# TFMV/hnsw

Hardware: AMD Instinct MI355X
Metric: queries/sec @ recall@10, 1M×768-d cosine; 1/2/4/8-GPU scaling (higher is better)
Workload: dtype fp32

## Files before the change

hnsw_amd/csrc/api.cpp:

```cpp
#include "index.hpp"

#include <functional>
#include <unordered_set>

using namespace mhh;

namespace mhh {

thread_local std::string g_create_err;

int fail(mhnsw_index* h, int code, const char* fmt, ...) {
    char buf[512];
    va_list ap;
    va_start(ap, fmt);
    vsnprintf(buf, sizeof(buf), fmt, ap);
    va_end(ap);
    if (h)
        h->err = buf;
    else
        g_create_err = buf;
    return code;
}

int validate(mhnsw_index* h) {
// ... 317 lines not shown
            h->ord_pin = nullptr;
            h->ord_cap = 0;
            if (hipHostMalloc((void**)&h->ord_pin, (size_t)nb * 4, hipHostMallocDefault) != hipSuccess)
                return fail(h, MHNSW_ENOMEM, "pinned allocation failed");
            h->ord_cap = nb;
        }
        if ((r = ensure_buf(h, h->border, (size_t)nb))) return r;
        if (h->ord_pending) HIPCHK(h, hipEventSynchronize(h->ord_ev));
        std::vector<int64_t> pos(MH_MAXL + 1, 0);
        for (int l = 0; l <= MH_MAXL; ++l) pos[l] = l < MH_MAXL ? count[l + 1] : 0;
        for (int64_t i = a0; i < a1; ++i)
            h->ord_pin[pos[std::min(h->hlevels[row_of(i)], MH_MAXL)]++] = (uint32_t)row_of(i);
        HIPCHK(h, hipMemcpyAsync(h->border.p, h->ord_pin, (size_t)nb * 4, hipMemcpyHostToDevice, h->stream));
        HIPCHK(h, hipEventRecord(h->ord_ev, h->stream));
        h->ord_pending = true;
    }
    auto vis16_for = [&](int ef) -> int {
        return h->vis_compact && ef > 128 && h->capn <= (int64_t(1) << 24) && h->vis_log2 == 12;
    };
    auto args = [&](int l) {
        const int mcap = l == 0 ? m0_of(h) : h->M;
        BatchBuildArgs a;
        a.order = nullptr;
        a.count = 0;
        a.g = graph_view(h);
        a.layer = l;
        a.n0 = rows ? 0 : a0;
        a.n1 = rows ? nb : a1;
        a.rows = rows ? h->border.p : nullptr;
        a.levels = h->levels;
// ... 30 lines not shown
        if (!h->time_build) return 0;
        if (h->ltev_used == h->ltev.size()) {
            hipEvent_t e;
            HIPCHK(h, hipEventCreate(&e));
            h->ltev.push_back(e);
        }
        HIPCHK(h, hipEventRecord(h->ltev[h->ltev_used++], h->stream));
        return 0;
    };
    for (int l = top; l >= 0; --l) {
        BatchBuildArgs a = args(l);
        const int mcap = a.mcap;
        if (fuse) {
            if (l == top) {
                if ((r = tmark())) return r;
                LCHK(h, launch_build_batch_descend(a, h->lpr, h->vpl, h->stream));
                if ((r = tmark())) return r;
            }
            if (l > maxlvl) continue;
            a.order = h->border.p;
            a.count = count[std::min(l, MH_MAXL)];
        }
        HIPCHK(h, hipMemsetAsync(h->touched_cnt, 0, 4, h->stream));
        if ((r = tmark())) return r;
        LCHK(h, launch_build_batch_search(a, h->lpr, h->vpl, h->stream));
        if (maxlvl >= l) LCHK(h, launch_build_batch_commit(a, h->lpr, h->vpl, (a1 - a0) * mcap, h->stream));
        if ((r = tmark())) return r;
        if (link && count[std::min(l, MH_MAXL)] >= 2) {
            if ((size_t)nb > h->link_cap || h->link_stride < h->layers[l].cap)
                return fail(h, MHNSW_EINTERNAL, "link staging too small");
            BatchBuildArgs la = a;
            la.ef = h->batch_link_ef > 0 ? std::min(std::max(h->batch_link_ef, mcap), 512) : a.ef;
            la.vis16 = vis16_for(la.ef);
            LinkArgs k;
            k.adj = h->link_adj;
            k.adjd = h->link_adjd;
// ... 564 lines not shown
        r = run_build_batch(h, n0, n1, top_live, entry_live, publish_keys);
        publish_keys();
    }
    HIPCHK(h, hipStreamSynchronize(h->stream));
    if (int rt = collect_build_times(h)) return rt;
    if (r == 0) *reached = nproc;
    *cont_out = cont;
    return r;
}

int add_impl(mhnsw_index* h, const int64_t* keys, const float* vecs, bool vecs_on_device, int64_t n, int dim,
             const int32_t* levels) {
    h->add_reached = 0;
    h->link_rows = h->link_edges = 0;
    h->link_us = 0;
    for (;;) {
        int64_t reached = 0, cont = -1;
        const int r = add_step(h, keys, vecs, vecs_on_device, n, dim, levels, &reached, &cont);
        h->add_reached += reached;
        if (r || cont <= 0 || cont >= n) return r;
        keys += cont;
        vecs += (size_t)cont * dim;
        n -= cont;
        if (levels) levels += cont;
    }
}

}

extern "C" {
// ... 76 lines not shown
        F(L.adj);
        F(L.adjd);
    }
    F(h->qpad.p);
    F(h->qnorm.p);
    F(h->scores.p);
    F(h->tmp.p);
    F(h->cand.p);
    F(h->border.p);
    F(h->okeys.p);
    F(h->odist.p);
    F(h->on.p);
    F(h->ordkey.p);
    F(h->ordval.p);
    F(h->ordtmp.p);
    F(h->nq.p);
    F(h->nneg.p);
    F(h->ncd.p);
    F(h->nck.p);
    F(h->nok.p);
    F(h->ncn.p);
    F(h->nci.p);
    F(h->noff.p);
    F(h->non.p);
    F(h->nos.p);
    F(h->xsplit.p);
    F(h->xinv.p);
    F(h->qinv.p);
    F(h->xerr.p);
    F(h->h1thr.p);
// ... 196 lines not shown
    } else if (n == "build_mw_max") {
        if (v < 0) return fail(h, MHNSW_EINVAL, "build_mw_max must be >= 0");
        h->build_mw_max = v;
    } else if (n == "beam_mw_max_b") {
        if (v < 0) return fail(h, MHNSW_EINVAL, "beam_mw_max_b must be >= 0");
        h->beam_mw_max_b = v;
    } else if (n == "beam_lds_min_ef") {
        if (v < 65 || v > 513) return fail(h, MHNSW_EINVAL, "beam_lds_min_ef must be in [65, 513]");
        h->beam_lds_min_ef = (int)v;
    } else if (n == "upper_ef") {
        if (v < 1 || v > 64) return fail(h, MHNSW_EINVAL, "upper_ef must be in [1, 64]");
        h->upper_ef = (int)v;
    } else if (n == "fuse_descent") {
        if (v != 0 && v != 1) return fail(h, MHNSW_EINVAL, "fuse_descent must be 0 or 1");
        h->fuse_descent = (int)v;
    } else if (n == "vis_compact") {
        if (v != 0 && v != 1) return fail(h, MHNSW_EINVAL, "vis_compact must be 0 or 1");
        h->vis_compact = (int)v;
    } else if (n == "filter_route") {
        if (v < 1 || v > 2048) return fail(h, MHNSW_EINVAL, "filter_route must be in [1, 2048]");
        h->filter_route = (int)v;
    } else if (n == "compact_stage_rows") {
        if (v < 1) return fail(h, MHNSW_EINVAL, "compact_stage_rows must be >= 1");
        h->compact_stage_rows = v;
    } else if (n == "time_build") {
        h->time_build = (int)(v != 0);
    } else if (n == "max_rows") {
        if (v < 0) return fail(h, MHNSW_EINVAL, "max_rows must be >= 0");
        h->max_rows = v;
    } else if (n == "screen") {
// ... 57 lines not shown
    else if (n == "batch_ratio_pct") *v = h->batch_ratio_pct;
    else if (n == "vis_log2") *v = h->vis_log2;
    else if (n == "vis_entries") *v = beam_vis_entries(h);
    else if (n == "exact_kk") *v = h->exact_kk;
    else if (n == "exact_sample") *v = h->exact_sample;
    else if (n == "exact_thr_rank") *v = h->exact_thr_rank;
    else if (n == "exact_precision") *v = h->exact_precision;
    else if (n == "exact_tile") *v = h->exact_tile;
    else if (n == "compat_waves") *v = h->compat_waves;
    else if (n == "upper_ef") *v = h->upper_ef;
    else if (n == "beam_mw_max_b") *v = h->beam_mw_max_b;
    else if (n == "beam_lds_min_ef") *v = h->beam_lds_min_ef;
    else if (n == "build_mw_max") *v = h->build_mw_max;
    else if (n == "screen") *v = h->screen;
    else if (n == "fuse_descent") *v = h->fuse_descent;
    else if (n == "vis_compact") *v = h->vis_compact;
    else if (n == "filter_route") *v = h->filter_route;
    else if (n == "time_build") *v = h->time_build;
    else if (n == "max_rows") *v = h->max_rows;
    else if (n == "strkey_relabels") *v = h->relabels;
    else if (n == "strkeys") *v = (int64_t)h->s2l.size();
    else if (n == "pitch") *v = h->pitch;
    else if (n == "capacity") *v = h->capn;
    else if (n == "last_gemm_ns") {
        float ms = 0.f;
        if (!h->have_gemm_timing || hipEventSynchronize(h->gev1) != hipSuccess ||
            hipEventElapsedTime(&ms, h->gev0, h->gev1) != hipSuccess)
            return MHNSW_EINVAL;
        *v = (int64_t)std::llround((double)ms * 1e6);
    }
// ... 485 lines not shown
    if (!relink && n > 0 && (!keys || !vecs || !out_found))
        return fail(h, MHNSW_EINVAL, "keys, vecs and out_found must be non-NULL");
    if (h->build_mode == MHNSW_BUILD_COMPAT || h->aliased || h->partial_rows > 0)
        return fail(h, MHNSW_EUNSUPPORTED, "update needs a batch or flat (build_mode 1 or 2) handle");
    if (n <= 0) return MHNSW_OK;
    if (!relink && h->layers_exist && dim != h->dim)
        return fail(h, MHNSW_EDIM, "embedding dimension mismatch: %d != %d", h->dim, dim);
    {
        std::unordered_set<int64_t> seen;
        seen.reserve((size_t)n);
        for (int64_t i = 0; i < n; ++i)
            if (!seen.insert(keys[i]).second)
                return fail(h, MHNSW_EINVAL, "duplicate key %lld in update", (long long)keys[i]);
    }
    h->update_rows = h->update_chunks = h->update_repaired = 0;
    h->update_us[0] = h->update_us[1] = h->update_us[2] = 0;
    std::vector<uint32_t> ids, from;
    for (int64_t i = 0; i < n; ++i) {
        out_found[i] = 0;
        auto it = h->key2id.find(keys[i]);
        if (it == h->key2id.end() || h->hdead[it->second] || !in_layer(h, it->second, 0)) continue;
        out_found[i] = 1;
        ids.push_back((uint32_t)it->second);
        from.push_back((uint32_t)i);
    }
    const int64_t m = (int64_t)ids.size();
    if (m == 0) return MHNSW_OK;
    ++h->mut_epoch;
    const bool flat = h->build_mode == MHNSW_BUILD_FLAT;
    hipStream_t s = h->stream;
// ... 437 lines not shown
```

hnsw_amd/csrc/beam.hpp:

```cpp
#pragma once
#include <type_traits>

#include "device_search.hpp"
#include "engine.hpp"

namespace mh {

template <int L, int V, int XW>
int launch_beam_cfg(const SearchArgs& a, hipStream_t s);
template <int L, int V, int XW>
int launch_beam_lds_cfg(const SearchArgs& a, hipStream_t s);
template <int L, int V>
int launch_beam_filt_cfg(const SearchArgs& a, const FilterArgs& f, hipStream_t s);

__host__ __device__ inline int beam_efl(const SearchArgs& a) { return a.ef > a.k ? a.ef : a.k; }
inline bool beam_in_lds(const SearchArgs& a) { return beam_efl(a) >= a.lds_min_ef; }

__host__ __device__ inline int beam_vis_words(const SearchArgs& a) { return a.vis16 ? VIS16_WORDS : a.vis_n; }

struct BeamLds {
    int list, words;
};
template <class LT>
__host__ __device__ inline BeamLds beam_lds(const SearchArgs& a) {
// ... 28 lines not shown
                const int32_t e = a.layer_entry[l];
                if (e < 0)
                    skip = true;
                else
                    ep = (uint32_t)e;
            }
            if (!skip) {
                beam_layer<C, 1, G, false, SCREEN, 1>(a.g, l, ep, a.upper_ef, q, qn, L1, smem, vsz, st, bev);
                float d;
                uint32_t id;
                bl_at(L1, 0, d, id);
                if (id != EMPTY_ID) ep = id & ID_MASK;
            }
            if constexpr (KEY) {
                if (l <= a.key_top && l > a.key_top - a.key_n) {
                    const uint32_t f = a.key_hash ? (ep * 2654435761u) >> (32 - a.key_id_bits)
                                                  : ep & ((1u << a.key_id_bits) - 1u);
                    *key = (*key << a.key_id_bits) | (unsigned long long)f;
                }
            }
        }
    }
    if (to0 && a.g.layers[0].deg[ep] == -2) ep = (uint32_t)a.layer_entry[0];
    return ep;
}

__device__ __forceinline__ uint32_t beam_entry_of(const SearchArgs& a, int64_t b) {
    return a.order ? uni(a.ep0[b]) : a.entry;
}
__device__ __forceinline__ int beam_entry_layer(const SearchArgs& a) { return a.order ? beam_order_lo(a) - 1 : a.top; }

__device__ __forceinline__ void beam_pad_out(const SearchArgs& a, int64_t b, int nvalid) {
    const int lane = lane_id();
// ... 58 lines not shown
        const bool ok = w != EMPTY_ID && !is_dead(a.g, id);
        const unsigned long long m = __ballot(ok);
        const int pos = nvalid + __popcll(m & below);
        if (ok && pos < a.k) {
            a.out_keys[b * a.k + pos] = a.g.keys[id];
            a.out_dist[b * a.k + pos] = bl_chunk_dist(L, c);
            if (a.out_ids) a.out_ids[b * a.k + pos] = (int32_t)id;
        }
        nvalid += __popcll(m);
    }
    beam_pad_out(a, b, min(nvalid, a.k));
}

__device__ __forceinline__ int64_t beam_query_of(const SearchArgs& a, int64_t i) {
    if (!a.order) return i < a.B ? i : -1;
    const int64_t pos = a.order_chunk > 0 ? (i & 7) * a.order_chunk + (i >> 3) : i;
    if (pos >= a.B || (a.order_chunk > 0 && (i >> 3) >= a.order_chunk)) return -1;
    const uint32_t b = uni(a.order[pos]);
    return b < (uint64_t)a.B ? (int64_t)b : -1;
}

__device__ __forceinline__ void beam_stats(const SearchArgs& a, const WaveStats& st) {
    if (lane_id() == 0) {
        atomicAdd(&a.stats[0], st.E);
        atomicAdd(&a.stats[1], st.X);
        if (st.resets) atomicAdd(&a.stats[2], st.resets);
        atomicAdd(&a.stats[8], st.S);
        atomicAdd(&a.stats[9], st.F);
#ifdef MH_PROF_BEAM
        atomicAdd(&a.stats[10], st.c_ins);
        atomicAdd(&a.stats[11], st.c_score);
// ... 212 lines not shown
```

hnsw_amd/csrc/build.hip:

```cpp
#include "build_batch.hpp"
#include "build_link.hpp"
#include "build_compat.hpp"

namespace mh {
#define X_(L, V, G)                                                                           \
    extern template int launch_build_compat_cfg<L, V>(const CompatBuildArgs&, int, hipStream_t); \
    extern template int launch_delete_compat_cfg<L, V>(const DeleteArgs&, hipStream_t);       \
    extern template int launch_batch_descend_cfg<L, V>(const BatchBuildArgs&, hipStream_t);   \
    extern template int launch_batch_search_cfg<L, V, 1>(const BatchBuildArgs&, hipStream_t); \
    extern template int launch_batch_search_cfg<L, V, 2>(const BatchBuildArgs&, hipStream_t); \
    extern template int launch_batch_search_cfg<L, V, 3>(const BatchBuildArgs&, hipStream_t); \
    extern template int launch_batch_search_cfg<L, V, 4>(const BatchBuildArgs&, hipStream_t); \
    extern template int launch_batch_commit_cfg<L, V>(const BatchBuildArgs&, int64_t, hipStream_t); \
    extern template int launch_batch_link_cfg<L, V, 1>(const BatchBuildArgs&, const LinkArgs&, hipStream_t); \
    extern template int launch_batch_link_cfg<L, V, 2>(const BatchBuildArgs&, const LinkArgs&, hipStream_t); \
    extern template int launch_batch_link_cfg<L, V, 3>(const BatchBuildArgs&, const LinkArgs&, hipStream_t); \
    extern template int launch_batch_link_cfg<L, V, 4>(const BatchBuildArgs&, const LinkArgs&, hipStream_t); \
    extern template int launch_delete_repair_cfg<L, V>(const DeleteArgs&, hipStream_t);
MH_FOR_EACH_CFG(X_)
#undef X_

int launch_build_compat(const CompatBuildArgs& a, int lpr, int vpl, int waves, hipStream_t s) {
    return with_cfg(lpr, vpl, [&](auto c) { return launch_build_compat_cfg<c.L, c.V>(a, waves, s); });
}
// ... 46 lines not shown
    if (keep) {
        c = k.adj[(size_t)slot * k.stride + lane];
        d = k.adjd[(size_t)slot * k.stride + lane];
        for (int j = 0; j < nin; ++j) keep = keep && a.inc_src[(size_t)u * a.inc_cap + j] != (uint32_t)c;
    }
    const unsigned long long m = __ballot(keep);
    if (keep) {
        const int e = __builtin_amdgcn_mbcnt_hi((uint32_t)(m >> 32), __builtin_amdgcn_mbcnt_lo((uint32_t)m, 0));
        a.g.layers[l].adj[(size_t)u * capl + e] = c;
        a.g.layers[l].adjd[(size_t)u * capl + e] = d;
    }
    if (lane == 0) a.g.layers[l].deg[u] = __popcll(m);
}

int launch_build_batch_link_apply(const BatchBuildArgs& a, const LinkArgs& k, hipStream_t s) {
    const int64_t n = a.order ? a.count : a.n1 - a.n0;
    if (n <= 0) return 0;
    return launch_grid(k_batch_link_apply, n, 64, 0, LinkKernelArgs{a, k}, s);
}

int launch_delete_compat(const DeleteArgs& a, int lpr, int vpl, hipStream_t s) {
    if (a.nids <= 0) return 0;
    return with_cfg(lpr, vpl, [&](auto c) { return launch_delete_compat_cfg<c.L, c.V>(a, s); });
}

int launch_delete_repair(const DeleteArgs& a, int lpr, int vpl, hipStream_t s) {
    if (a.n <= 0) return 0;
    return with_cfg(lpr, vpl, [&](auto c) { return launch_delete_repair_cfg<c.L, c.V>(a, s); });
}

}
// ... 1 lines not shown
```

hnsw_amd/csrc/build_batch.hpp:

```cpp
#pragma once
#include <algorithm>
#include <type_traits>

#include "device_search.hpp"
#include "engine.hpp"

namespace mh {

template <int L, int V>
int launch_batch_descend_cfg(const BatchBuildArgs& a, hipStream_t s);
template <int L, int V, int XW>
int launch_batch_search_cfg(const BatchBuildArgs& a, hipStream_t s);
template <int L, int V>
int launch_batch_commit_cfg(const BatchBuildArgs& a, int64_t max_touched, hipStream_t s);
template <int L, int V>
int launch_delete_repair_cfg(const DeleteArgs& a, hipStream_t s);

template <class C, int G, int NR>
__device__ __forceinline__ void drop_pass(const GraphDev& g, const QReg<C>& qr, float rn, int pos,
                                          uint32_t live, uint32_t& dropped, const uint32_t (&ids)[NR],
                                          const float (&ed)[NR], float alpha, float margin, WaveStats& st) {
    const int lane = lane_id();
    const bool scr = h16_query_ok(rn);
    st.F += 1;
// ... 43 lines not shown
                ++k;
            });
            const int dks = __shfl((int)dk, du, 64);
            dr = dr || (und && dks != 0);
        }
        const int drs = __shfl((int)dr, dst, 64);
        if (cand && drs != 0) dropped |= 1u << r;
    }
}

__device__ __forceinline__ int batch_vsize(const BatchBuildArgs& a) { return a.vis16 ? -1 : 1 << a.vis_log2; }
__host__ __device__ inline int batch_vis_words(const BatchBuildArgs& a) {
    return a.vis16 ? std::max(1 << a.vis_log2, VIS16_WORDS) : 1 << a.vis_log2;
}

template <class C, int G, bool SCREEN>
__global__ __launch_bounds__(64) void k_batch_descend(BatchBuildArgs a) {
    extern __shared__ __attribute__((aligned(16))) uint32_t smem[];
    const int64_t u64 = a.n0 + blockIdx.x;
    if (u64 >= a.n1) return;
    const uint32_t u = a.rows ? a.rows[u64] : (uint32_t)u64;
    const int lv = a.levels[u];
    if (lv >= a.layer) return;
    WaveStats st;
    QReg<C> q;
    load_query(q, a.g.vecs + (size_t)u * a.g.pitch);
    const float qn = a.g.norms[u];
    uint32_t ep = a.cur_entry[u];
    for (int l = a.layer; l > lv; --l) {
        BList<1> L1;
        beam_layer<C, 1, G, false, SCREEN>(a.g, l, ep, 1, q, qn, L1, smem, batch_vsize(a), st);
        float d;
        uint32_t id;
        bl_at(L1, 0, d, id);
        if (id != EMPTY_ID) ep = id & ID_MASK;
    }
    if (lane_id() == 0) {
        a.cur_entry[u] = ep;
        atomicAdd(&a.stats[0], st.E);
        atomicAdd(&a.stats[1], st.X);
        atomicAdd(&a.stats[6], st.S);
        atomicAdd(&a.stats[7], st.F);
    }
}

template <class C, int R, int G, bool SCREEN>
__device__ __forceinline__ int select_neighbours(const BatchBuildArgs& a, const BList<R>& L, int nl, uint32_t& sel,
                                                 float& seld, WaveStats& st) {
    const int lane = lane_id();
    bool sel_screen = false;
    float margin = 0.f;
// ... 127 lines not shown
        if (lane == 0) a.g.layers[l].deg[u] = nsel;
    }
}

__device__ __forceinline__ void batch_stats(const BatchBuildArgs& a, const WaveStats& st) {
    if (lane_id() == 0) {
        atomicAdd(&a.stats[0], st.E);
        atomicAdd(&a.stats[1], st.X);
        atomicAdd(&a.stats[6], st.S);
        atomicAdd(&a.stats[7], st.F);
    }
}

__device__ __forceinline__ bool batch_node(const BatchBuildArgs& a, uint32_t& u) {
    if (a.order) {
        if (blockIdx.x >= a.count) return false;
        u = a.order[blockIdx.x];
    } else {
        const int64_t u64 = a.n0 + blockIdx.x;
        if (u64 >= a.n1) return false;
        u = a.rows ? a.rows[u64] : (uint32_t)u64;
    }
    return true;
}

template <class C, int R, int G, bool SCREEN, int XW>
__global__ __launch_bounds__(64, MH_BUILD_WPS) void k_batch_search(BatchBuildArgs a) {
    extern __shared__ __attribute__((aligned(16))) uint32_t smem[];
    uint32_t u;
    if (!batch_node(a, u)) return;
    WaveStats st;
    QReg<C> q;
// ... 278 lines not shown
        rowd[lane] = keptd;
    }
    if (lane == 0) {
        a.g.layers[l].deg[v] = nkeep;
        atomicAdd(&a.stats[0], st.E);
        if (a.repaired) atomicAdd(a.repaired, 1ull);
    }
}

template <int L, int V>
int launch_batch_descend_cfg(const BatchBuildArgs& a, hipStream_t s) {
    using C = Cfg<L, V>;
    constexpr int G = cfg_group<L, V>();
    const int64_t n = a.n1 - a.n0;
    if (n <= 0) return 0;
    return a.g.h16 ? launch_grid(k_batch_descend<C, G, true>, n, 64, batch_vis_words(a), a, s)
                   : launch_grid(k_batch_descend<C, G, false>, n, 64, batch_vis_words(a), a, s);
}

template <class F>
int batch_with_list(int ef, F&& f) {
    if (ef <= 64) return f(std::integral_constant<int, 1>());
    if (ef <= 128) return f(std::integral_constant<int, 2>());
    if (ef <= 256) return f(std::integral_constant<int, 4>());
    if (ef <= 512) return f(std::integral_constant<int, 8>());
    return -4;
}

#ifndef MH_BUILD_GMAX
#define MH_BUILD_GMAX 8
#endif

template <int L, int V, int XW>
int launch_batch_search_cfg(const BatchBuildArgs& a, hipStream_t s) {
    using C = Cfg<L, V>;
    constexpr int G = std::min(cfg_group<L, V>(), MH_BUILD_GMAX);
    return batch_with_list(a.ef, [&](auto regs) {
        constexpr int R = decltype(regs)::value;
        const int lds_mw = batch_vis_words(a);
        const int lds = lds_mw + (R >= 4 ? BL_MERGE_WORDS : 0);
        const int64_t n = a.order ? a.count : a.n1 - a.n0;
        if (n <= 0) return 0;
        if constexpr (XW >= 2) {
            if (a.g.h16 && n <= a.mw_max)
                return launch_grid(k_batch_search_mw<C, R, G, true, XW>, n, 64 * BMW_WAVES, lds_mw, a, s);
        }
        return a.g.h16 ? launch_grid(k_batch_search<C, R, G, true, XW>, n, 64, lds, a, s)
                       : launch_grid(k_batch_search<C, R, G, false, XW>, n, 64, lds, a, s);
    });
}

template <int L, int V>
int launch_batch_commit_cfg(const BatchBuildArgs& a, int64_t max_touched, hipStream_t s) {
    constexpr int G = std::min(cfg_group<L, V>(), 4);
    return launch_grid(k_batch_commit<Cfg<L, V>, G>, std::min<int64_t>(max_touched, 32768), 64, 0, a, s);
}

template <int L, int V>
int launch_delete_repair_cfg(const DeleteArgs& a, hipStream_t s) {
    constexpr int G = std::min(cfg_group<L, V>(), 4);
    return launch_grid(k_delete_repair<Cfg<L, V>, G>, a.n, 64, 0, a, s);
}

// ... 2 lines not shown
```

hnsw_amd/csrc/build_link.hpp:

```cpp
#pragma once
#include "build_batch.hpp"

namespace mh {

template <int L, int V, int XW>
int launch_batch_link_cfg(const BatchBuildArgs& a, const LinkArgs& k, hipStream_t s);

struct LinkKernelArgs {
    BatchBuildArgs a;
    LinkArgs k;
};

template <class C, int R, int G, bool SCREEN, int XW>
__global__ __launch_bounds__(64, MH_BUILD_WPS) void k_batch_link(LinkKernelArgs ka) {
    const BatchBuildArgs& a = ka.a;
    const LinkArgs& k = ka.k;
    extern __shared__ __attribute__((aligned(16))) uint32_t smem[];
    uint32_t u;
    if (!batch_node(a, u)) return;
    const int l = a.layer;
    if (a.levels[u] < l) return;
    const int lane = lane_id();
    const int64_t slot = (int64_t)u - a.n0;
    WaveStats st;
// ... 58 lines not shown
            k.deg[slot] = nsel;
            atomicAdd(&k.cnt[0], 1ull);
            atomicAdd(&k.cnt[1], (unsigned long long)__popcll(mnew));
        }
    }
    batch_stats(a, st);
}

template <int L, int V, int XW>
int launch_batch_link_cfg(const BatchBuildArgs& a, const LinkArgs& k, hipStream_t s) {
    using C = Cfg<L, V>;
    constexpr int G = std::min(cfg_group<L, V>(), MH_BUILD_GMAX);
    return batch_with_list(a.ef, [&](auto regs) {
        constexpr int R = decltype(regs)::value;
        const int lds = batch_vis_words(a) + (R >= 4 ? BL_MERGE_WORDS : 0);
        const int64_t n = a.order ? a.count : a.n1 - a.n0;
        if (n <= 0) return 0;
        const LinkKernelArgs p{a, k};
        return a.g.h16 ? launch_grid(k_batch_link<C, R, G, true, XW>, n, 64, lds, p, s)
                       : launch_grid(k_batch_link<C, R, G, false, XW>, n, 64, lds, p, s);
    });
}

}
```

hnsw_amd/csrc/engine.hpp:

```cpp
#pragma once
#include <hip/hip_runtime.h>
#include <stdint.h>

#include "device_common.hpp"

namespace mh {

struct DimCfgId {
    int lpr, vpl;
};
inline bool pick_cfg(int dim, int& lpr, int& vpl) {
    if (dim <= 0) return false;
    if (dim <= 64) { lpr = 16; vpl = 1; return true; }
    if (dim <= 128) { lpr = 32; vpl = 1; return true; }
    if (dim <= 256) { lpr = 64; vpl = 1; return true; }
    if (dim <= 512) { lpr = 64; vpl = 2; return true; }
    if (dim <= 768) { lpr = 64; vpl = 3; return true; }
    if (dim <= 1024) { lpr = 64; vpl = 4; return true; }
    if (dim <= 1536) { lpr = 64; vpl = 6; return true; }
    if (dim <= 2048) { lpr = 64; vpl = 8; return true; }
    if (dim <= 3072) { lpr = 64; vpl = 12; return true; }
    if (dim <= 4096) { lpr = 64; vpl = 16; return true; }
    return false;
}
// ... 58 lines not shown
    uint32_t* oidx = nullptr;
    uint32_t* pstat = nullptr;
    int key_top = 0, key_n = 0;
    int key_id_bits = 1;
    int key_hash = 0;
    int64_t order_chunk = 0;
};

struct FilterArgs {
    const uint32_t* const* filters;
    int nslots;
    int ef;
    const int32_t* filter_of;
};

inline bool beam_small_batch(const SearchArgs& a) {
    const int efl = a.ef > a.k ? a.ef : a.k;
    return a.expand != 2 && a.expand != 4 && efl <= 128 && efl < a.lds_min_ef && a.B <= a.mw_max_b;
}
inline int64_t beam_order_grid(const SearchArgs& a) { return a.order_chunk > 0 ? 8 * a.order_chunk : a.B; }

struct NegArgs {
    GraphDev g;
    const float* neg;
    const int32_t* neg_off;
    const int32_t* cand_ids;
    const float* cand_d;
    const int32_t* cand_n;
    int64_t B;
    int kx, k;
// ... 77 lines not shown
    int expand;
    float alpha;
    int32_t* inc_cnt;
    uint32_t* inc_src;
    float* inc_dist;
    int inc_cap;
    uint32_t* touched;
    int32_t* touched_cnt;
    unsigned long long* stats;
    int vis_log2;
    const uint32_t* order;
    int64_t count;
    int64_t mw_max = 0;
    int vis16 = 0;
    const uint32_t* rows = nullptr;
};
int launch_build_batch_search(const BatchBuildArgs& a, int lpr, int vpl, hipStream_t s);
int launch_build_batch_descend(const BatchBuildArgs& a, int lpr, int vpl, hipStream_t s);
int launch_build_batch_commit(const BatchBuildArgs& a, int lpr, int vpl, int64_t n_touched, hipStream_t s);
struct LinkArgs {
    int32_t* adj;
    float* adjd;
    int32_t* deg;
    int stride;
    unsigned long long* cnt;
};
int launch_build_batch_link(const BatchBuildArgs& a, const LinkArgs& k, int lpr, int vpl, hipStream_t s);
int launch_build_batch_link_apply(const BatchBuildArgs& a, const LinkArgs& k, hipStream_t s);

struct ExactArgs {
    const float* X;
// ... 171 lines not shown
```

hnsw_amd/csrc/index.hpp:

```cpp
#pragma once
#include <hip/hip_runtime.h>

#include <errno.h>
#include <fcntl.h>
#include <unistd.h>

#include <algorithm>
#include <cmath>
#include <cstdarg>
#include <cstdio>
#include <cstring>
#include <map>
#include <mutex>
#include <shared_mutex>
#include <string>
#include <functional>
#include <unordered_map>
#include <vector>

#include "../../include/mhnsw.h"
#include "codec.hpp"
#include "engine.hpp"

using namespace mh;

#ifndef MH_SEARCH_ORDER_DEFAULT
#define MH_SEARCH_ORDER_DEFAULT 1
#endif
#ifndef MH_SEARCH_ORDER_MIN_B_DEFAULT
#define MH_SEARCH_ORDER_MIN_B_DEFAULT 16384
#endif

namespace mhh {

template <class T>
struct DevBuf {
    T* p = nullptr;
    size_t n = 0;
};

struct Layer {
    int32_t* deg = nullptr;
    int32_t* adj = nullptr;
    float* adjd = nullptr;
    int cap = 0;
// ... 30 lines not shown
    int exact_thr_rank = 0;
    int exact_precision = 3;
    int exact_tile = 0;
    int compat_waves = 8;
    int upper_ef = 1;
    int64_t beam_mw_max_b = 512;
    int beam_lds_min_ef = 513;
    int search_order = MH_SEARCH_ORDER_DEFAULT;
    int64_t search_order_min_b = MH_SEARCH_ORDER_MIN_B_DEFAULT;
    int search_order_top = 0;
    int search_order_fields = 0;
    int search_order_map = 0;
    int64_t build_mw_max = 256;
    int screen = 1;
    int fuse_descent = 1;
    int time_build = 0;
    int batch_link = 0;
    int batch_link_ef = 0;
    int64_t max_rows = 0;
    std::vector<hipEvent_t> tev;
    size_t tev_used = 0;
    std::vector<hipEvent_t> ltev;
    size_t ltev_used = 0;
    double build_search_us = 0;
    int32_t* link_adj = nullptr;
    float* link_adjd = nullptr;
    int32_t* link_deg = nullptr;
    size_t link_cap = 0;
    int link_stride = 0;
    unsigned long long* link_cnt = nullptr;
// ... 33 lines not shown
    int* d_err = nullptr;
    std::vector<mhh::Layer> layers;
    DevBuf<float> qpad, qnorm, scores, tmp;
    DevBuf<uint32_t> cand;
    DevBuf<uint32_t> border;
    uint32_t* ord_pin = nullptr;
    int64_t ord_cap = 0;
    hipEvent_t ord_ev = nullptr;
    bool ord_pending = false;
    DevBuf<int64_t> okeys;
    DevBuf<float> odist;
    DevBuf<int32_t> on;
    DevBuf<unsigned long long> ordkey;
    DevBuf<uint32_t> ordval;
    DevBuf<uint8_t> ordtmp;
    DevBuf<float> nq, nneg, ncd;
    DevBuf<int64_t> nck, nok;
    DevBuf<int32_t> ncn, nci, noff, non;
    DevBuf<float> nos;
    DevBuf<uint16_t> xsplit, qsplit;
    int64_t xsplit_rows = 0, xsplit_plane = 0;
    int xsplit_kind = 0;
    DevBuf<float> xinv, qinv;
    DevBuf<float> xerr;
    DevBuf<float> h1thr, h1c, h1s, qerr;
    DevBuf<float> h1xw;
    DevBuf<uint2> h1region, h1bucket;
    DevBuf<int32_t> h1rcnt, h1qcnt;
    DevBuf<uint8_t> h1ovf;
    DevBuf<float> xbound, xmaxn, xsegd;
// ... 117 lines not shown
int collect_build_times(mhnsw_index* h);
int run_build_batch(mhnsw_index* h, int64_t n0, int64_t n1, int top, uint32_t entry,
                    const std::function<void()>& while_gpu = nullptr);
int h16_rows(mhnsw_index* h, int64_t r0, int64_t r1);
int32_t kid_of_row(const mhnsw_index* h, int64_t r);
int set_kidlive(mhnsw_index* h, int32_t kid, int32_t row);
int start_alias(mhnsw_index* h);
void forget_key(mhnsw_index* h, int64_t key, int32_t row);
std::vector<int32_t> key_rows(const mhnsw_index* h, int64_t key);
int32_t key_row_in(const mhnsw_index* h, int64_t key, int l);
int add_step(mhnsw_index* h, const int64_t* keys, const float* vecs, bool vecs_on_device, int64_t n, int dim, const int32_t* levels, int64_t* reached, int64_t* cont_out);
int add_impl(mhnsw_index* h, const int64_t* keys, const float* vecs, bool vecs_on_device, int64_t n, int dim, const int32_t* levels);
int beam_vis_entries(const mhnsw_index* h);
int drain(mhnsw_index* h);
int search_impl(mhnsw_index* h, const float* queries, bool on_device, int64_t B, int dim, int k, int mode, int ef, const int64_t* entry_key, int64_t* okeys, float* odist, int32_t* on, hipStream_t s, bool timing, int32_t* out_ids = nullptr, bool sticky = false);
int device_error(mhnsw_index* h, int err);
void reset_graph(mhnsw_index* h);
constexpr int MHNSW_MAX_FILTERS = 1024;
void drop_filters(mhnsw_index* h);
int filters_fit(mhnsw_index* h);
int search_filtered_impl(mhnsw_index* h, const float* queries, bool on_device, int64_t B, int dim, int k, int ef, int route, const int32_t* filter_of, int64_t* okeys, float* odist, int32_t* on, hipStream_t s, bool sticky);
int search_filtered_exact_impl(mhnsw_index* h, const float* queries, bool on_device, int64_t B, int dim, int k, int filter, int64_t* okeys, float* odist, int32_t* on, hipStream_t s, bool sticky);
int range_search_impl(mhnsw_index* h, const float* queries, int64_t B, int dim, const float* radius, int mode, int ef, int64_t* out_lims);
int range_search_device_impl(mhnsw_index* h, const float* d_queries, int64_t B, int dim, const float* d_radius, int mode, int ef, int64_t cap, int64_t* d_lims, int64_t* d_keys, float* d_dist, hipStream_t s);
int range_search_filtered_impl(mhnsw_index* h, const float* queries, int64_t B, int dim, const float* radius, int mode, int ef, int route, const int32_t* filter_of, int64_t* out_lims);
int range_search_filtered_device_impl(mhnsw_index* h, const float* d_queries, int64_t B, int dim, const float* d_radius, int mode, int ef, int route, int filter, int64_t cap, int64_t* d_lims, int64_t* d_keys, float* d_dist, hipStream_t s);
int import_csr(mhnsw_index* h, int64_t N, int dim, int L, int cap, const int64_t* keys, const float* vecs, const int32_t* deg, const int32_t* adj, const int32_t* entry, const uint8_t* dead);
const char* metric_name(int m);
int strkey_relabel(mhnsw_index* h);
int strkey_insert(mhnsw_index* h, const std::string& s);
// ... 39 lines not shown
```

hnsw_amd/csrc/search_host.cpp:

```cpp
#include "index.hpp"

using namespace mhh;

namespace mhh {

int beam_vis_entries(const mhnsw_index* h) {
    if (h->vis_entries > 0) return h->vis_entries;
    return std::min(32768, 5 << (h->vis_log2 - 2));
}

int drain(mhnsw_index* h) {
    if (h->scr_valid) HIPCHK(h, hipEventSynchronize(h->scr_ev));
    h->scr_valid = false;
    return 0;
}

int device_error(mhnsw_index* h, int err) {
    if (!err) return 0;
    if (err & 4) return fail(h, MHNSW_EINTERNAL, "out-of-range node id in adjacency (graph corrupt)");
    if (err & 8) return fail(h, MHNSW_EINVAL, "unknown filter in filter_of");
    return fail(h, MHNSW_EINTERNAL, "visited set overflow (raise vis_log2)");
}

struct SearchCall {
// ... 107 lines not shown
    a.stats = h->d_stats;
    a.err = c.errw;
    a.vis_log2 = h->vis_log2;
    a.vis_n = beam_vis_entries(h);
    a.vis16 = h->vis_compact && width > 128 && h->capn <= (int64_t(1) << 24) &&
              (int64_t)a.vis_n >= (int64_t)VIS16_WORDS && a.vis_n < VIS16_HOMES;
    if (lds_tier && !a.vis16 && h->vis_entries <= 0) a.vis_n = std::max(a.vis_n, 4 * std::min(width, 2048));
    a.upper_ef = h->upper_ef;
    a.mw_max_b = h->beam_mw_max_b;
    a.expand = h->search_expand;
    return 0;
}

constexpr int ORDER_KEY_FIELDS = 3;
constexpr int64_t ORDER_CELL_QUERIES = 128;
static void order_key_layers(const mhnsw_index* h, int64_t B, int top, SearchArgs& a) {
    int bits = 1;
    while (bits < 31 && (int64_t(1) << bits) < h->capn) ++bits;
    int kt = h->search_order_top;
    if (kt <= 0) {
        kt = 1;
        while (kt < top && h->layers[kt].count > std::max<int64_t>(1, B / ORDER_CELL_QUERIES)) ++kt;
    }
    a.key_top = std::min(kt, top);
    a.key_n = std::min(h->search_order_fields > 0 ? h->search_order_fields : ORDER_KEY_FIELDS, a.key_top);
    a.key_id_bits = a.key_n > 0 ? std::min(bits, 64 / a.key_n) : 1;
    a.key_hash = a.key_id_bits < bits;
}

static int beam_search(mhnsw_index* h, const SearchCall& c, SearchArgs& a) {
    int r;
    const int64_t B = c.B;
    hipStream_t s = c.s;
    if (std::max(a.ef, a.k) > 2048) return fail(h, MHNSW_EUNSUPPORTED, "beam mode supports max(ef,k) <= 2048");
    a.lds_min_ef = h->beam_lds_min_ef;
    const bool ordered = h->search_order && B >= h->search_order_min_b && !beam_small_batch(a);
    size_t tmp_bytes = 0;
    if (ordered) {
        LCHK(h, order_sort_temp_bytes(B, &tmp_bytes));
        const size_t pstat_at = ((size_t)3 * B + 3) & ~(size_t)3;
        if ((r = ensure_buf(h, h->ordkey, (size_t)2 * B)) || (r = ensure_buf(h, h->ordval, pstat_at + (size_t)4 * B)) ||
            (r = ensure_buf(h, h->ordtmp, std::max<size_t>(tmp_bytes, 1))))
            return r;
        a.okey = h->ordkey.p;
        a.oidx = h->ordval.p;
        a.ep0 = h->ordval.p + 2 * B;
        a.pstat = h->ordval.p + pstat_at;
        order_key_layers(h, B, a.top, a);
        a.order_chunk = h->search_order_map == 0 ? (B + 7) / 8 : 0;
    }
    if (c.timing) HIPCHK(h, hipEventRecord(h->ev0, s));
    int lr = 0;
    if (ordered && !(lr = launch_beam_descend(a, h->lpr, h->vpl, s))) {
        LCHK(h, launch_order_sort(h->ordkey.p, h->ordkey.p + B, h->ordval.p, h->ordval.p + B, B,
                                  a.key_n * a.key_id_bits, h->ordtmp.p, tmp_bytes, s));
        a.order = h->ordval.p + B;
    }
    if (!lr) lr = launch_search_beam(a, h->lpr, h->vpl, s);
    if (lr == -2)
        return fail(h, MHNSW_EUNSUPPORTED, "beam search LDS budget exceeded (ef=%d, k=%d, vis_entries=%d)", a.ef, a.k,
                    a.vis_n);
    LCHK(h, lr);
    if (c.timing) HIPCHK(h, hipEventRecord(h->ev1, s));
    return 0;
// ... 999 lines not shown
```

Before: 2.947 million.

## Sort batch-build layer-0 nodes by upper-layer descent path for locality

During fused batch build, the descend kernel now emits a sort key for each inserted node, built from the entry points it visited in the upper layers (plus its own id for layers it occupies). A radix sort then reorders the layer-0 search and commit work so that nodes with similar entry paths run in adjacent blocks, with an optional XCD-chunked mapping. This reuses the query-ordering scheme from search and aims to improve cache locality of graph and vector reads during construction. It adds a sort pass and extra buffers, and it only affects build time, not the query path being measured.

```diff
diff --git a/hnsw_amd/csrc/api.cpp b/hnsw_amd/csrc/api.cpp
--- a/hnsw_amd/csrc/api.cpp
+++ b/hnsw_amd/csrc/api.cpp
@@ -355,6 +355,20 @@
         HIPCHK(h, hipMemcpyAsync(h->border.p, h->ord_pin, (size_t)nb * 4, hipMemcpyHostToDevice, h->stream));
         HIPCHK(h, hipEventRecord(h->ord_ev, h->stream));
         h->ord_pending = true;
+    }
+    const bool ordered = fuse && h->build_order != 0 && nb >= h->build_order_min_b;
+    OrderKey okl;
+    size_t sort_bytes = 0;
+    if (ordered) {
+        const int64_t cap = std::max<int64_t>(nb, std::min<int64_t>(h->batch_max, 65536));
+        size_t cap_bytes = 0;
+        LCHK(h, order_sort_temp_bytes(cap, &cap_bytes));
+        LCHK(h, order_sort_temp_bytes(nb, &sort_bytes));
+        if ((r = ensure_buf(h, h->bordkey, (size_t)2 * cap)) || (r = ensure_buf(h, h->bordval, (size_t)2 * cap)) ||
+            (r = ensure_buf(h, h->bordtmp, std::max<size_t>(std::max(cap_bytes, sort_bytes), 1))))
+            return r;
+        okl = order_key_layers(h, nb, top);
+        ++h->build_ordered;
     }
     auto vis16_for = [&](int ef) -> int {
         return h->vis_compact && ef > 128 && h->capn <= (int64_t(1) << 24) && h->vis_log2 == 12;
@@ -415,12 +429,26 @@
         if (fuse) {
             if (l == top) {
                 if ((r = tmark())) return r;
+                if (ordered) {
+                    a.okey = h->bordkey.p;
+                    a.oval = h->bordval.p;
+                    a.key = okl;
+                }
                 LCHK(h, launch_build_batch_descend(a, h->lpr, h->vpl, h->stream));
+                if (ordered)
+                    LCHK(h, launch_order_sort(h->bordkey.p, h->bordkey.p + nb, h->bordval.p, h->bordval.p + nb, nb,
+                                              okl.n * okl.id_bits, h->bordtmp.p, sort_bytes, h->stream));
+                a.okey = nullptr;
+                a.oval = nullptr;
                 if ((r = tmark())) return r;
             }
             if (l > maxlvl) continue;
             a.order = h->border.p;
             a.count = count[std::min(l, MH_MAXL)];
+            if (ordered && l == 0) {
+                a.order = h->bordval.p + nb;
+                a.order_chunk = h->build_order_map == 0 ? xcd_chunk_of(nb) : 0;
+            }
         }
         HIPCHK(h, hipMemsetAsync(h->touched_cnt, 0, 4, h->stream));
         if ((r = tmark())) return r;
@@ -1015,6 +1043,7 @@
     h->add_reached = 0;
     h->link_rows = h->link_edges = 0;
     h->link_us = 0;
+    h->build_ordered = 0;
     for (;;) {
         int64_t reached = 0, cont = -1;
         const int r = add_step(h, keys, vecs, vecs_on_device, n, dim, levels, &reached, &cont);
@@ -1121,6 +1150,9 @@
     F(h->ordkey.p);
     F(h->ordval.p);
     F(h->ordtmp.p);
+    F(h->bordkey.p);
+    F(h->bordval.p);
+    F(h->bordtmp.p);
     F(h->nq.p);
     F(h->nneg.p);
     F(h->ncd.p);
@@ -1347,6 +1379,15 @@
     } else if (n == "fuse_descent") {
         if (v != 0 && v != 1) return fail(h, MHNSW_EINVAL, "fuse_descent must be 0 or 1");
         h->fuse_descent = (int)v;
+    } else if (n == "build_order") {
+        if (v != 0 && v != 1) return fail(h, MHNSW_EINVAL, "build_order must be 0 or 1");
+        h->build_order = (int)v;
+    } else if (n == "build_order_min_b") {
+        if (v < 1) return fail(h, MHNSW_EINVAL, "build_order_min_b must be >= 1");
+        h->build_order_min_b = v;
+    } else if (n == "build_order_map") {
+        if (v != 0 && v != 1) return fail(h, MHNSW_EINVAL, "build_order_map must be 0 or 1");
+        h->build_order_map = (int)v;
     } else if (n == "vis_compact") {
         if (v != 0 && v != 1) return fail(h, MHNSW_EINVAL, "vis_compact must be 0 or 1");
         h->vis_compact = (int)v;
@@ -1434,6 +1475,10 @@
     else if (n == "build_mw_max") *v = h->build_mw_max;
     else if (n == "screen") *v = h->screen;
     else if (n == "fuse_descent") *v = h->fuse_descent;
+    else if (n == "build_order") *v = h->build_order;
+    else if (n == "build_order_min_b") *v = h->build_order_min_b;
+    else if (n == "build_order_map") *v = h->build_order_map;
+    else if (n == "last_build_ordered") *v = h->build_ordered;
     else if (n == "vis_compact") *v = h->vis_compact;
     else if (n == "filter_route") *v = h->filter_route;
     else if (n == "time_build") *v = h->time_build;
@@ -1949,6 +1994,7 @@
                 return fail(h, MHNSW_EINVAL, "duplicate key %lld in update", (long long)keys[i]);
     }
     h->update_rows = h->update_chunks = h->update_repaired = 0;
+    h->build_ordered = 0;
     h->update_us[0] = h->update_us[1] = h->update_us[2] = 0;
     std::vector<uint32_t> ids, from;
     for (int64_t i = 0; i < n; ++i) {
diff --git a/hnsw_amd/csrc/beam.hpp b/hnsw_amd/csrc/beam.hpp
--- a/hnsw_amd/csrc/beam.hpp
+++ b/hnsw_amd/csrc/beam.hpp
@@ -66,9 +66,7 @@
             }
             if constexpr (KEY) {
                 if (l <= a.key_top && l > a.key_top - a.key_n) {
-                    const uint32_t f = a.key_hash ? (ep * 2654435761u) >> (32 - a.key_id_bits)
-                                                  : ep & ((1u << a.key_id_bits) - 1u);
-                    *key = (*key << a.key_id_bits) | (unsigned long long)f;
+                    *key = order_key_push(*key, ep, a.key_id_bits, a.key_hash);
                 }
             }
         }
@@ -157,7 +155,7 @@
 
 __device__ __forceinline__ int64_t beam_query_of(const SearchArgs& a, int64_t i) {
     if (!a.order) return i < a.B ? i : -1;
-    const int64_t pos = a.order_chunk > 0 ? (i & 7) * a.order_chunk + (i >> 3) : i;
+    const int64_t pos = a.order_chunk > 0 ? xcd_chunk_pos(i, a.order_chunk) : i;
     if (pos >= a.B || (a.order_chunk > 0 && (i >> 3) >= a.order_chunk)) return -1;
     const uint32_t b = uni(a.order[pos]);
     return b < (uint64_t)a.B ? (int64_t)b : -1;
diff --git a/hnsw_amd/csrc/build.hip b/hnsw_amd/csrc/build.hip
--- a/hnsw_amd/csrc/build.hip
+++ b/hnsw_amd/csrc/build.hip
@@ -84,7 +84,7 @@
 }
 
 int launch_build_batch_link_apply(const BatchBuildArgs& a, const LinkArgs& k, hipStream_t s) {
-    const int64_t n = a.order ? a.count : a.n1 - a.n0;
+    const int64_t n = batch_grid(a);
     if (n <= 0) return 0;
     return launch_grid(k_batch_link_apply, n, 64, 0, LinkKernelArgs{a, k}, s);
 }
diff --git a/hnsw_amd/csrc/build_batch.hpp b/hnsw_amd/csrc/build_batch.hpp
--- a/hnsw_amd/csrc/build_batch.hpp
+++ b/hnsw_amd/csrc/build_batch.hpp
@@ -81,14 +81,26 @@
     return a.vis16 ? std::max(1 << a.vis_log2, VIS16_WORDS) : 1 << a.vis_log2;
 }
 
-template <class C, int G, bool SCREEN>
+template <class C, int G, bool SCREEN, bool KEY>
 __global__ __launch_bounds__(64) void k_batch_descend(BatchBuildArgs a) {
     extern __shared__ __attribute__((aligned(16))) uint32_t smem[];
     const int64_t u64 = a.n0 + blockIdx.x;
     if (u64 >= a.n1) return;
     const uint32_t u = a.rows ? a.rows[u64] : (uint32_t)u64;
     const int lv = a.levels[u];
-    if (lv >= a.layer) return;
+    const int key_lo = a.key.top - a.key.n;
+    unsigned long long key = 0;
+    auto own_fields = [&](int l_hi) {
+        for (int l = min(l_hi, a.key.top); l > key_lo; --l) key = order_key_push(key, u, a.key.id_bits, a.key.hash);
+        if (lane_id() == 0) {
+            a.okey[u64 - a.n0] = key;
+            a.oval[u64 - a.n0] = u;
+        }
+    };
+    if (lv >= a.layer) {
+        if constexpr (KEY) own_fields(a.layer);
+        return;
+    }
     WaveStats st;
     QReg<C> q;
     load_query(q, a.g.vecs + (size_t)u * a.g.pitch);
@@ -101,7 +113,11 @@
         uint32_t id;
         bl_at(L1, 0, d, id);
         if (id != EMPTY_ID) ep = id & ID_MASK;
-    }
+        if constexpr (KEY) {
+            if (l <= a.key.top && l > key_lo) key = order_key_push(key, ep, a.key.id_bits, a.key.hash);
+        }
+    }
+    if constexpr (KEY) own_fields(lv);
     if (lane_id() == 0) {
         a.cur_entry[u] = ep;
         atomicAdd(&a.stats[0], st.E);
@@ -259,8 +275,14 @@
 
 __device__ __forceinline__ bool batch_node(const BatchBuildArgs& a, uint32_t& u) {
     if (a.order) {
-        if (blockIdx.x >= a.count) return false;
-        u = a.order[blockIdx.x];
+        int64_t pos = blockIdx.x;
+        if (a.order_chunk > 0) {
+            if ((pos >> 3) >= a.order_chunk) return false;
+            pos = xcd_chunk_pos(pos, a.order_chunk);
+        }
+        if (pos >= a.count) return false;
+        u = a.order[pos];
+        if (a.rows ? u >= a.g.capn : ((int64_t)u < a.n0 || (int64_t)u >= a.n1)) return false;
     } else {
         const int64_t u64 = a.n0 + blockIdx.x;
         if (u64 >= a.n1) return false;
@@ -569,8 +591,11 @@
     constexpr int G = cfg_group<L, V>();
     const int64_t n = a.n1 - a.n0;
     if (n <= 0) return 0;
-    return a.g.h16 ? launch_grid(k_batch_descend<C, G, true>, n, 64, batch_vis_words(a), a, s)
-                   : launch_grid(k_batch_descend<C, G, false>, n, 64, batch_vis_words(a), a, s);
+    if (a.okey && a.oval)
+        return a.g.h16 ? launch_grid(k_batch_descend<C, G, true, true>, n, 64, batch_vis_words(a), a, s)
+                       : launch_grid(k_batch_descend<C, G, false, true>, n, 64, batch_vis_words(a), a, s);
+    return a.g.h16 ? launch_grid(k_batch_descend<C, G, true, false>, n, 64, batch_vis_words(a), a, s)
+                   : launch_grid(k_batch_descend<C, G, false, false>, n, 64, batch_vis_words(a), a, s);
 }
 
 template <class F>
@@ -596,12 +621,13 @@
         const int lds = lds_mw + (R >= 4 ? BL_MERGE_WORDS : 0);
         const int64_t n = a.order ? a.count : a.n1 - a.n0;
         if (n <= 0) return 0;
+        const int64_t grid = batch_grid(a);
         if constexpr (XW >= 2) {
             if (a.g.h16 && n <= a.mw_max)
-                return launch_grid(k_batch_search_mw<C, R, G, true, XW>, n, 64 * BMW_WAVES, lds_mw, a, s);
-        }
-        return a.g.h16 ? launch_grid(k_batch_search<C, R, G, true, XW>, n, 64, lds, a, s)
-                       : launch_grid(k_batch_search<C, R, G, false, XW>, n, 64, lds, a, s);
+                return launch_grid(k_batch_search_mw<C, R, G, true, XW>, grid, 64 * BMW_WAVES, lds_mw, a, s);
+        }
+        return a.g.h16 ? launch_grid(k_batch_search<C, R, G, true, XW>, grid, 64, lds, a, s)
+                       : launch_grid(k_batch_search<C, R, G, false, XW>, grid, 64, lds, a, s);
     });
 }
 
diff --git a/hnsw_amd/csrc/build_link.hpp b/hnsw_amd/csrc/build_link.hpp
--- a/hnsw_amd/csrc/build_link.hpp
+++ b/hnsw_amd/csrc/build_link.hpp
@@ -96,7 +96,7 @@
     return batch_with_list(a.ef, [&](auto regs) {
         constexpr int R = decltype(regs)::value;
         const int lds = batch_vis_words(a) + (R >= 4 ? BL_MERGE_WORDS : 0);
-        const int64_t n = a.order ? a.count : a.n1 - a.n0;
+        const int64_t n = batch_grid(a);
         if (n <= 0) return 0;
         const LinkKernelArgs p{a, k};
         return a.g.h16 ? launch_grid(k_batch_link<C, R, G, true, XW>, n, 64, lds, p, s)
diff --git a/hnsw_amd/csrc/engine.hpp b/hnsw_amd/csrc/engine.hpp
--- a/hnsw_amd/csrc/engine.hpp
+++ b/hnsw_amd/csrc/engine.hpp
@@ -96,6 +96,20 @@
     const int32_t* filter_of;
 };
 
+__host__ __device__ inline int64_t xcd_chunk_of(int64_t n) { return (n + 7) / 8; }
+__host__ __device__ inline int64_t xcd_chunk_pos(int64_t i, int64_t chunk) { return (i & 7) * chunk + (i >> 3); }
+
+struct OrderKey {
+    int top = 0, n = 0;
+    int id_bits = 1;
+    int hash = 0;
+};
+__host__ __device__ inline unsigned long long order_key_push(unsigned long long key, uint32_t id, int id_bits,
+                                                             int hash) {
+    const uint32_t f = hash ? (id * 2654435761u) >> (32 - id_bits) : id & ((1u << id_bits) - 1u);
+    return (key << id_bits) | (unsigned long long)f;
+}
+
 inline bool beam_small_batch(const SearchArgs& a) {
     const int efl = a.ef > a.k ? a.ef : a.k;
     return a.expand != 2 && a.expand != 4 && efl <= 128 && efl < a.lds_min_ef && a.B <= a.mw_max_b;
@@ -203,7 +217,14 @@
     int64_t mw_max = 0;
     int vis16 = 0;
     const uint32_t* rows = nullptr;
-};
+    unsigned long long* okey = nullptr;
+    uint32_t* oval = nullptr;
+    OrderKey key;
+    int64_t order_chunk = 0;
+};
+inline int64_t batch_grid(const BatchBuildArgs& a) {
+    return a.order ? (a.order_chunk > 0 ? 8 * a.order_chunk : a.count) : a.n1 - a.n0;
+}
 int launch_build_batch_search(const BatchBuildArgs& a, int lpr, int vpl, hipStream_t s);
 int launch_build_batch_descend(const BatchBuildArgs& a, int lpr, int vpl, hipStream_t s);
 int launch_build_batch_commit(const BatchBuildArgs& a, int lpr, int vpl, int64_t n_touched, hipStream_t s);
diff --git a/hnsw_amd/csrc/index.hpp b/hnsw_amd/csrc/index.hpp
--- a/hnsw_amd/csrc/index.hpp
+++ b/hnsw_amd/csrc/index.hpp
@@ -29,6 +29,15 @@
 #endif
 #ifndef MH_SEARCH_ORDER_MIN_B_DEFAULT
 #define MH_SEARCH_ORDER_MIN_B_DEFAULT 16384
+#endif
+#ifndef MH_BUILD_ORDER_DEFAULT
+#define MH_BUILD_ORDER_DEFAULT 1
+#endif
+#ifndef MH_BUILD_ORDER_MIN_B_DEFAULT
+#define MH_BUILD_ORDER_MIN_B_DEFAULT 4096
+#endif
+#ifndef MH_BUILD_ORDER_MAP_DEFAULT
+#define MH_BUILD_ORDER_MAP_DEFAULT 1
 #endif
 
 namespace mhh {
@@ -89,6 +98,10 @@
     int64_t build_mw_max = 256;
     int screen = 1;
     int fuse_descent = 1;
+    int build_order = MH_BUILD_ORDER_DEFAULT;
+    int64_t build_order_min_b = MH_BUILD_ORDER_MIN_B_DEFAULT;
+    int build_order_map = MH_BUILD_ORDER_MAP_DEFAULT;
+    int64_t build_ordered = 0;
     int time_build = 0;
     int batch_link = 0;
     int batch_link_ef = 0;
@@ -152,6 +165,9 @@
     DevBuf<unsigned long long> ordkey;
     DevBuf<uint32_t> ordval;
     DevBuf<uint8_t> ordtmp;
+    DevBuf<unsigned long long> bordkey;
+    DevBuf<uint32_t> bordval;
+    DevBuf<uint8_t> bordtmp;
     DevBuf<float> nq, nneg, ncd;
     DevBuf<int64_t> nck, nok;
     DevBuf<int32_t> ncn, nci, noff, non;
@@ -299,6 +315,7 @@
 int beam_vis_entries(const mhnsw_index* h);
 int drain(mhnsw_index* h);
 int search_impl(mhnsw_index* h, const float* queries, bool on_device, int64_t B, int dim, int k, int mode, int ef, const int64_t* entry_key, int64_t* okeys, float* odist, int32_t* on, hipStream_t s, bool timing, int32_t* out_ids = nullptr, bool sticky = false);
+OrderKey order_key_layers(const mhnsw_index* h, int64_t B, int top);
 int device_error(mhnsw_index* h, int err);
 void reset_graph(mhnsw_index* h);
 constexpr int MHNSW_MAX_FILTERS = 1024;
diff --git a/hnsw_amd/csrc/search_host.cpp b/hnsw_amd/csrc/search_host.cpp
--- a/hnsw_amd/csrc/search_host.cpp
+++ b/hnsw_amd/csrc/search_host.cpp
@@ -145,7 +145,7 @@
 
 constexpr int ORDER_KEY_FIELDS = 3;
 constexpr int64_t ORDER_CELL_QUERIES = 128;
-static void order_key_layers(const mhnsw_index* h, int64_t B, int top, SearchArgs& a) {
+OrderKey order_key_layers(const mhnsw_index* h, int64_t B, int top) {
     int bits = 1;
     while (bits < 31 && (int64_t(1) << bits) < h->capn) ++bits;
     int kt = h->search_order_top;
@@ -153,10 +153,12 @@
         kt = 1;
         while (kt < top && h->layers[kt].count > std::max<int64_t>(1, B / ORDER_CELL_QUERIES)) ++kt;
     }
-    a.key_top = std::min(kt, top);
-    a.key_n = std::min(h->search_order_fields > 0 ? h->search_order_fields : ORDER_KEY_FIELDS, a.key_top);
-    a.key_id_bits = a.key_n > 0 ? std::min(bits, 64 / a.key_n) : 1;
-    a.key_hash = a.key_id_bits < bits;
+    OrderKey k;
+    k.top = std::max(std::min(kt, top), 0);
+    k.n = std::min(h->search_order_fields > 0 ? h->search_order_fields : ORDER_KEY_FIELDS, k.top);
+    k.id_bits = k.n > 0 ? std::min(bits, 64 / k.n) : 1;
+    k.hash = k.id_bits < bits;
+    return k;
 }
 
 static int beam_search(mhnsw_index* h, const SearchCall& c, SearchArgs& a) {
@@ -177,8 +179,12 @@
         a.oidx = h->ordval.p;
         a.ep0 = h->ordval.p + 2 * B;
         a.pstat = h->ordval.p + pstat_at;
-        order_key_layers(h, B, a.top, a);
-        a.order_chunk = h->search_order_map == 0 ? (B + 7) / 8 : 0;
+        const OrderKey ok = order_key_layers(h, B, a.top);
+        a.key_top = ok.top;
+        a.key_n = ok.n;
+        a.key_id_bits = ok.id_bits;
+        a.key_hash = ok.hash;
+        a.order_chunk = h->search_order_map == 0 ? xcd_chunk_of(B) : 0;
     }
     if (c.timing) HIPCHK(h, hipEventRecord(h->ev0, s));
     int lr = 0;
```

New measurement: 2.933 million. About the same (-0.5%).
